# yjtang249/MIPSFusion

Measured on AMD Instinct MI355X. Metric: rays*samples/s per GPU, full optimisation iteration (fwd + bwd + pose+map Adam), 4096 rays x 64 samples, 640x480 RGB-D, higher is better.
Workload: dtype f32; decoder products as 3 x bf16 pieces of each fp32 operand, 6 bf16 MFMAs per product, fp32 accumulate; 1 GPU; BASELINE config 2: FastCaMo-synth apartment_2, 1 active submap per GPU, 4096 rays x 64 samples, hash grid 2^19 x 16 x 2, 620x460 synthetic RGB-D; rays=4096, samples_per_ray=64, hash_size=19, parallelism=single gpu

## Files before the change

include/mipsf.h:

```cpp
#ifndef MIPSF_H
#define MIPSF_H

#include <stdint.h>

#ifdef __cplusplus
extern "C" {
#endif

#define MIPSF_MAX_LEVELS 32
#define MIPSF_ABI_VERSION 2

const char* mipsf_last_error(void);
int mipsf_abi_version(void);
int mipsf_device_cu_count(void);

typedef struct mipsf_grid_meta {
    uint32_t n_levels;
    uint32_t n_features;
    uint32_t log2_hashmap_size;
    uint32_t base_resolution;
    float per_level_scale;
    float log2_per_level_scale;
    uint32_t n_params;
    uint32_t offsets[MIPSF_MAX_LEVELS + 1];
// ... 115 lines not shown
    uint32_t struct_size;
    uint32_t M;
    const float* packed16;
    const float* x;
    const float* out;
    const float* dout;
    const float* saved;
    float* dfeat;
    float* dx;
    float* dact;
    uint32_t* tile_live;
    int feat_layout;
    int flags;
    uint32_t packed16_floats;
    const uint32_t* live_list;
} mipsf_decoder_chain16_args;
int mipsf_decoder_bwd_chain16(const mipsf_decoder_chain16_args* args_host, void* stream);
#define MIPSF_WGRAD_LEAN_DACT 1u
#define MIPSF_WGRAD_DETERMINISTIC 2u
#define MIPSF_TILE_ORDER_MAX_M (1u << 27)
typedef struct mipsf_decoder_wgrad16_args {
    uint32_t struct_size;
    uint32_t M;
    const float* packed16;
    const float* feat;
    const float* x;
    const float* saved;
    const float* dact;
    const uint32_t* tile_live;
    const mipsf_decoder_grads* grads;
// ... 156 lines not shown
```

mipsfusion_amd/_lib.py:

```python
from __future__ import annotations

import ctypes as C
import os
from typing import Optional

import torch

_HERE = os.path.dirname(os.path.abspath(__file__))
LIB_PATH = os.environ.get("MIPSF_LIB") or os.path.join(_HERE, "libmipsf_hip.so")
MAX_LEVELS = 32
FEAT_AOS, FEAT_LEVEL_MAJOR = 0, 1
PREC = {"f32": 0, "f16x3": 1, "f16": 2, "bf16x3": 3, "bf16x6": 4}


class GridMeta(C.Structure):
    _fields_ = [("n_levels", C.c_uint32), ("n_features", C.c_uint32), ("log2_hashmap_size", C.c_uint32),
                ("base_resolution", C.c_uint32), ("per_level_scale", C.c_float),
                ("log2_per_level_scale", C.c_float), ("n_params", C.c_uint32),
                ("offsets", C.c_uint32 * (MAX_LEVELS + 1)), ("resolutions", C.c_uint32 * MAX_LEVELS),
                ("scales", C.c_float * MAX_LEVELS)]


class DecoderWeights(C.Structure):
    _fields_ = [(n, C.c_void_p) for n in ("w_pts0", "b_pts0", "w_pts2", "b_pts2", "w_rgb0", "b_rgb0",
# ... 21 lines not shown
        return a
    cls.new = staticmethod(new)
    return cls


_VP, _CU, _CI = C.c_void_p, C.c_uint32, C.c_int
HashgridBwdArgs = _args("HashgridBwdArgs", [("M", _CU), ("x", _VP), ("params", _VP), ("dout", _VP), ("dparams", _VP), ("dx", _VP),
                                            ("scratch", _VP), ("counters", _VP), ("meta", C.POINTER(GridMeta)),
                                            ("feat_layout", _CI), ("flags", _CU)])
DecoderFwd16Args = _args("DecoderFwd16Args", [("M", _CU), ("packed16", _VP), ("feat", _VP), ("x", _VP), ("out", _VP), ("saved", _VP),
                                              ("tile_live_clear", _VP), ("feat_layout", _CI), ("precision", _CI),
                                              ("sdf_only", _CI), ("lean_record", _CI), ("packed16_floats", _CU)])
DecoderChain16Args = _args("DecoderChain16Args", [("M", _CU), ("packed16", _VP), ("x", _VP), ("out", _VP), ("dout", _VP),
                                                  ("saved", _VP), ("dfeat", _VP), ("dx", _VP), ("dact", _VP), ("tile_live", _VP),
                                                  ("feat_layout", _CI), ("flags", _CI), ("packed16_floats", _CU),
                                                  ("live_list", _VP)])
DecoderWgrad16Args = _args("DecoderWgrad16Args", [("M", _CU), ("packed16", _VP), ("feat", _VP), ("x", _VP), ("saved", _VP),
                                                  ("dact", _VP), ("tile_live", _VP), ("grads", C.POINTER(DecoderGrads)),
                                                  ("partial", _VP), ("feat_layout", _CI), ("arithmetic", _CI), ("flags", _CU),
                                                  ("packed16_floats", _CU), ("live_list", _VP)])
RenderFwdArgs = _args("RenderFwdArgs", [("N", _CU), ("S", _CU), ("raw", _VP), ("z_vals", _VP), ("target_rgb", _VP), ("target_d", _VP),
                                        ("counts", _VP), ("cfg", C.POINTER(RenderCfg)), ("rgb", _VP), ("depth", _VP),
                                        ("depth_var", _VP), ("disp", _VP), ("acc", _VP), ("weights", _VP), ("losses", _VP),
                                        ("partial", _VP), ("loss_weights", _VP), ("loss_total", _VP), ("ticket", _VP),
                                        ("sums", _VP), ("draw", _VP)])
RenderBwdArgs = _args("RenderBwdArgs", [("N", _CU), ("S", _CU), ("N_norm", _CU), ("raw", _VP), ("z_vals", _VP), ("target_rgb", _VP),
                                        ("target_d", _VP), ("counts", _VP), ("losses", _VP), ("cfg", C.POINTER(RenderCfg)),
                                        ("g_losses", _VP), ("g_total", _VP), ("loss_weights", _VP), ("g_rgb", _VP),
                                        ("g_depth", _VP), ("draw", _VP), ("flags", _CU)])
RENDER_BWD_KEEP_IF_UNIT = 1

# ... 535 lines not shown
```

mipsfusion_amd/csrc/common.h:

```cpp
#pragma once
#include <hip/hip_runtime.h>
#include <stdint.h>
#include <stdarg.h>
#include <stdio.h>

#include "../../include/mipsf.h"
#include "../../include/mipsf_compact.h"

#define MIPSF_WAVE 64

namespace mipsf {

void set_error(const char* fmt, ...);
int check_launch(const char* what);

constexpr int MAX_DEVICES = 64;
inline int device_slot() {
    int d = 0;
    if (hipGetDevice(&d) != hipSuccess || d < 0 || d >= MAX_DEVICES) return 0;
    return d;
}
int device_cus();

uint64_t hashgrid_bwd_scratch_floats(const mipsf_grid_meta* meta, uint32_t M, int need_dx);
// ... 56 lines not shown
    }
    n.norm_factor = c.norm_factor;
    return n;
}

#if defined(__HIP_DEVICE_COMPILE__) && !defined(MIPSF_KEEP_PACKED_FP32)
#define MIPSF_SINGLE_FP32 __attribute__((target("no-packed-fp32-ops")))
#else
#define MIPSF_SINGLE_FP32
#endif

__device__ __forceinline__ float normalise1(float p, double sub, double div, double nf) {
    return (float)((((double)p - sub) / div) / nf);
}

__device__ __forceinline__ float wave_sum(float v) {
#pragma unroll
    for (int o = 32; o > 0; o >>= 1) v += __shfl_xor(v, o, 64);
    return v;
}
__device__ __forceinline__ double wave_sum_d(double v) {
#pragma unroll
    for (int o = 32; o > 0; o >>= 1) v += __shfl_xor(v, o, 64);
    return v;
}

__device__ __forceinline__ float sigmoidf_(float x) { return 1.0f / (1.0f + expf(-x)); }

}
```

mipsfusion_amd/csrc/decoder16.hip:

```cpp
#include "decoder_dev.h"
#include "launch.h"
#include <stdlib.h>

namespace mipsf {
using namespace dl;

typedef _Float16 h8 __attribute__((ext_vector_type(8)));
typedef _Float16 h2 __attribute__((ext_vector_type(2)));
typedef __bf16 bf8 __attribute__((ext_vector_type(8)));
typedef __bf16 bf2 __attribute__((ext_vector_type(2)));

__device__ __forceinline__ f32x16 mfma16(h8 a, h8 b, f32x16 c) {
    return __builtin_amdgcn_mfma_f32_32x32x16_f16(a, b, c, 0, 0, 0);
}
template <int NP>
__device__ __forceinline__ f32x16 mfmaP(h8 a, h8 b, f32x16 c) {
    if constexpr (NP == 3)
        return __builtin_amdgcn_mfma_f32_32x32x16_bf16(__builtin_bit_cast(bf8, a), __builtin_bit_cast(bf8, b), c, 0, 0, 0);
    else
        return __builtin_amdgcn_mfma_f32_32x32x16_f16(a, b, c, 0, 0, 0);
}

template <bool SPLIT>
__device__ __forceinline__ void split8(const float (&v)[8], h8& hi, h8& lo) {
// ... 752 lines not shown
    const uint32_t lo = wbits[2 * w], hi = wbits[2 * w + 1];
    const uint64_t s = (uint64_t)blockIdx.x * LC_BLOCK + t;
    const bool live = ((lane < 32 ? lo >> lane : hi >> (lane - 32)) & 1u) != 0u && s < M;
    pos += lane < 32 ? (uint32_t)__popc(lo & ((1u << lane) - 1u)) : (uint32_t)__popc(lo) + (uint32_t)__popc(hi & ((1u << (lane - 32)) - 1u));
    if (live) ll[MIPSF_LIVE_HEADER + pos] = (uint32_t)s;
    if (blockIdx.x == gridDim.x - 1) {
        uint32_t total = 0;
        for (uint32_t v = 0; v < LC_BLOCK / MIPSF_WAVE; ++v) total += wsum[v];
        for (uint32_t v = 0; v < LC_BLOCK / 32; ++v) total += (uint32_t)__popc(wbits[v]);
        const uint32_t padded = (total + 31u) & ~31u;
        if (t < padded - total) ll[MIPSF_LIVE_HEADER + total + t] = MIPSF_LIVE_PAD;
        if (t == 0) ll[0] = total, ll[1] = padded / 32u;
    }
}

template <int LAYOUT, int NP, bool COMPACT = false, typename Img>
__device__ __forceinline__ void decoder16_bwd_tile(const Img bimg, const float* __restrict__ x,
                                                   const float* __restrict__ out, const float* __restrict__ dout,
                                                   const float* __restrict__ saved, float* __restrict__ dfeat,
                                                   float* __restrict__ dx, float* __restrict__ dact,
                                                   float* __restrict__ dsmall, uint32_t M, int64_t tile, int lane_in,
                                                   uint32_t* __restrict__ tile_live = nullptr, bool lean_dact = false,
                                                   const uint32_t* __restrict__ live_idx = nullptr) {
    static_assert(NP == 2 || NP == 3, "the chain runs on split operands");
    int lane = lane_in;
    asm volatile("" : "+v"(lane));
    const int j = lane & 31, h = lane >> 5;
    const uint32_t s_raw = COMPACT ? live_idx[tile * 32 + j] : (uint32_t)(tile * 32 + j);
    const bool live = s_raw < M;
    const uint32_t s = live ? s_raw : M - 1;
    const uint32_t lane16 = 16u * (uint32_t)lane;
    const srd_t da = make_srd(dact ? dact + (size_t)tile * ACT_TILE_FLOATS : nullptr, dact ? ACT_TILE_FLOATS * 4 : 0);
    const srd_t da_opt = make_srd(dact ? dact + (size_t)tile * ACT_TILE_FLOATS : nullptr, (dact && !lean_dact) ? ACT_TILE_FLOATS * 4 : 0);

#ifdef D16_TRACE
    unsigned long long tr_t[12];
    const unsigned long long tr_w0 = wall_clock64();
#endif
// ... 29 lines not shown
    }
    D16_MARK(1);
    {
        const float2* o = reinterpret_cast<const float2*>(out + (size_t)s * 10);
#pragma unroll
        for (int c = 0; c < 5; ++c) o2[c] = o[c];
    }
#ifndef D16_BWD_X_LATE
    const float x0 = x[3 * (size_t)s], x1 = x[3 * (size_t)s + 1], x2 = x[3 * (size_t)s + 2];
#endif
    const uint2* mk = reinterpret_cast<const uint2*>(saved + (((size_t)M + 127) / 128) * 4 * ACT_TILE_FLOATS) +
                      (COMPACT ? (size_t)(s >> 5) * (MASK_TILE_WORDS / 2) + ((s & 31u) + 32u * (uint32_t)h)
                               : (size_t)tile * (MASK_TILE_WORDS / 2) + lane);
    const uint2 mk1 = mk[0], mk3 = mk[64];
    const uint32_t m1[2] = {mk1.x, mk1.y}, m3[2] = {mk3.x, mk3.y};

    D16_MARK(2);
    float dlg[N_CLASS], drgb[3];
    {
        const float gv[10] = {g2[0].x, g2[0].y, g2[1].x, g2[1].y, g2[2].x, g2[2].y, g2[3].x, g2[3].y, g2[4].x, g2[4].y};
        const float ov[10] = {o2[0].x, o2[0].y, o2[1].x, o2[1].y, o2[2].x, o2[2].y, o2[3].x, o2[3].y, o2[4].x, o2[4].y};
        const float g_sdf = live ? gv[3] : 0.f, g_ent = live ? gv[4] : 0.f;
        float p[N_CLASS], dp[N_CLASS], dot = 0.f;
#pragma unroll
        for (int c = 0; c < N_CLASS; ++c) {
            p[c] = ov[5 + c];
            const float q = p[c] + 1e-5f;
            const float dent = -1.0f * (log2f(q) + p[c] / (q * 0.69314718055994530942f));
            dp[c] = (live ? gv[5 + c] : 0.f) + g_sdf * (0.5f * (float)c) + g_ent * dent;
            dot += p[c] * dp[c];
// ... 36 lines not shown
        buf_store16_nosoff<D16_BWD_STORE_AUX>((mat == 2 || (mat == 1 && q >= 8)) ? da_opt : da, lane16, (mat * 16 + q) * 1024,
                           make_float4(acc[rt][4 * g] * down, acc[rt][4 * g + 1] * down, acc[rt][4 * g + 2] * down,
                                       acc[rt][4 * g + 3] * down));
    };

    D16_MARK(3);
    f32x16 dG3[4];
    mfma16_layer<RT16_S2T, T16_S2T, NP, INIT_ZERO>(bimg.at(OFF16B_S2T, OFF16B_S2T), lane, h, dG3,
        [&](int, h8 (&b)[3]) { b[0] = lgp[0], b[1] = lgp[1], b[2] = lgp[2]; });
#pragma unroll
    for (int rt = 0; rt < 4; ++rt)
#pragma unroll
        for (int r = 0; r < 16; ++r) dG3[rt][r] = mask_apply(m3, rt, r, dG3[rt][r] * acc_unscale<NP>());

    D16_MARK(4);
    f32x16 dIn3[3];
    mfma16_layer<RT16_B3, T16_B3, NP, INIT_ZERO>(bimg.at(OFF16B_B3, OFF16B_B3), lane, h, dIn3,
        [&](int t, h8 (&b)[3]) {
            float v[8];
#pragma unroll
            for (int u = 0; u < 8; ++u) v[u] = dG3[t >> 1][8 * (t & 1) + u];
            cut8<NP>(v, b);
        },
        [&](int t) {
            store_piece(2, dG3, 2 * t);
            store_piece(2, dG3, 2 * t + 1);
        });
#pragma unroll
    for (int rt = 0; rt < 3; ++rt)
#pragma unroll
        for (int r = 0; r < 16; ++r) dIn3[rt][r] = dIn3[rt][r] * acc_unscale<NP>();
    if (live) {
#pragma unroll
        for (int r = 0; r < 16; r += 2) {
            const int row = rowmap(r, h);
            const float2 v = make_float2(dIn3[2][r] * down, dIn3[2][r + 1] * down);
            if (LAYOUT == MIPSF_FEAT_AOS)
                *reinterpret_cast<float2*>(dfeat + (size_t)s * N_GRID + row) = v;
            else
                *reinterpret_cast<float2*>(dfeat + ((size_t)(row >> 1) * M + s) * 2) = v;
        }
    }

    D16_MARK(5);
    f32x16 dH2[4];
    dH2[0] = dIn3[0], dH2[1] = dIn3[1];
    {
        f32x16 dRgb[2];
        mfma16_layer<RT16_RGBT, T16_RGBT, NP, INIT_ZERO>(bimg.at(OFF16B_RGBT, OFF16B_RGBT), lane, h, dRgb,
            [&](int, h8 (&b)[3]) { b[0] = rgp[0], b[1] = rgp[1], b[2] = rgp[2]; });
        dH2[2] = dRgb[0] * acc_unscale<NP>(), dH2[3] = dRgb[1] * acc_unscale<NP>();
    }

    D16_MARK(6);
    f32x16 dG1[4];
    mfma16_layer<RT16_B2, T16_B2, NP, INIT_ZERO>(bimg.at(OFF16B_B2, OFF16B_B2), lane, h, dG1,
// ... 1 lines not shown
            float v[8];
#pragma unroll
            for (int u = 0; u < 8; ++u) v[u] = dH2[t >> 1][8 * (t & 1) + u];
            cut8<NP>(v, b);
        },
        [&](int t) {
            store_piece(1, dH2, 2 * t);
            store_piece(1, dH2, 2 * t + 1);
        });
#pragma unroll
    for (int rt = 0; rt < 4; ++rt)
#pragma unroll
        for (int r = 0; r < 16; ++r) dG1[rt][r] = mask_apply(m1, rt, r, dG1[rt][r] * acc_unscale<NP>());

    D16_MARK(7);
    f32x16 dE[2];
    mfma16_layer<RT16_B1, T16_B1, NP, INIT_ZERO>(bimg.at(OFF16B_B1, OFF16B_B1), lane, h, dE,
        [&](int t, h8 (&b)[3]) {
            if (t == 8) {
                b[0] = rgp[0], b[1] = rgp[1], b[2] = rgp[2];
            } else {
                float v[8];
#pragma unroll
                for (int u = 0; u < 8; ++u) v[u] = dG1[(t >> 1) & 3][8 * (t & 1) + u];
                cut8<NP>(v, b);
            }
        },
        [&](int t) {
            if (t < 8) {
                store_piece(0, dG1, 2 * t);
// ... 11 lines not shown
    float g3[3] = {0.f, 0.f, 0.f};
#pragma unroll
    for (int d = 0; d < 3; ++d) {
        const float xd = d == 0 ? x0 : (d == 1 ? x1 : x2);
#pragma unroll
        for (int k = 0; k < 8; ++k) {
            const float arg = fmaf(ldexpf(xd, k), PI_F, h ? HALF_PI_F : 0.0f);
            g3[d] = g3[d] + de[d * 8 + k] * ((ldexpf(1.0f, k) * PI_F) * cos_reduced(arg));
        }
    }
    g3[0] += h == 0 ? de[24] : 0.0f;
    g3[1] += h == 1 ? de[24] : 0.0f;
    g3[2] += h == 0 ? de[25] : 0.0f;
#pragma unroll
    for (int d = 0; d < 3; ++d) g3[d] = g3[d] + __shfl_xor(g3[d], 32, 64);
    if (live && h == 0) {
        dx[3 * (size_t)s] = g3[0], dx[3 * (size_t)s + 1] = g3[1], dx[3 * (size_t)s + 2] = g3[2];
    }
#ifdef D16_TRACE
    D16_MARK(9);
    if (lane == 0) {
        const unsigned w = (blockIdx.x * (blockDim.x >> 6) + (threadIdx.x >> 6)) & 4095u;
        for (int k = 0; k < 9; ++k) d16_trace[w * 16 + k] += tr_t[k + 1] - tr_t[k];
        d16_trace[w * 16 + 12] += wall_clock64() - tr_w0;
        d16_trace[w * 16 + 15] += 1ull;
    }
#endif
}

template <int LAYOUT, int NP, bool COMPACT>
__global__ __launch_bounds__(DEC_BLOCK, 2) void decoder16_bwd_kernel(const float* __restrict__ packed16,
                                                                     const float* __restrict__ x,
                                                                     const float* __restrict__ out,
                                                                     const float* __restrict__ dout,
                                                                     const float* __restrict__ saved,
                                                                     float* __restrict__ dfeat, float* __restrict__ dx,
                                                                     float* __restrict__ dact, float* __restrict__ dsmall,
                                                                     uint32_t M, uint32_t* __restrict__ tile_live, uint32_t lean_dact,
                                                                     const uint32_t* __restrict__ live_list) {
    const int lane = threadIdx.x & 63;
    const int64_t tile = (int64_t)blockIdx.x * (DEC_BLOCK / 64) + __builtin_amdgcn_readfirstlane((int)(threadIdx.x >> 6));
    if (tile * 32 >= (int64_t)M) return;
    if (COMPACT && tile >= (int64_t)live_list[1]) return;
    const ImgBuf bimg{make_srd(reinterpret_cast<const _Float16*>(packed16 + TAIL16_FLOATS) + OFF16_BWD_HALVES,
                               IMG16B_HALVES * 4), 0u, (uint32_t)IMG16B_HALVES * 2u, ext16_srd<NP>(packed16), (uint32_t)EXT16_BWD * 2u};
    decoder16_bwd_tile<LAYOUT, NP, COMPACT>(bimg, x, out, dout, saved, dfeat, dx, dact, dsmall, M, tile, lane, tile_live, lean_dact != 0u,
                                            COMPACT ? live_list + MIPSF_LIVE_HEADER : nullptr);
}

constexpr int B16_LDS_BYTES = IMG16B_HALVES * 4;
static_assert(B16_LDS_BYTES <= 160 * 1024, "the backward image sets must fit the LDS of a CU");
template <int LAYOUT, int NP, bool COMPACT>
__global__ __launch_bounds__(F16_LDS_BLOCK, 1) void decoder16_bwd_lds_kernel(const float* __restrict__ packed16,
                                                                             const float* __restrict__ x,
                                                                             const float* __restrict__ out,
                                                                             const float* __restrict__ dout,
                                                                             const float* __restrict__ saved,
                                                                             float* __restrict__ dfeat,
                                                                             float* __restrict__ dx,
                                                                             float* __restrict__ dact,
                                                                             float* __restrict__ dsmall, uint32_t M,
                                                                             uint32_t n_tiles_all,
                                                                             uint32_t* __restrict__ tile_live, uint32_t lean_dact,
                                                                             const uint32_t* __restrict__ live_list) {
    const uint32_t n_tiles = COMPACT ? (uint32_t)__builtin_amdgcn_readfirstlane((int)live_list[1]) : n_tiles_all;
    const uint32_t* live_idx = COMPACT ? live_list + MIPSF_LIVE_HEADER : nullptr;
    extern __shared__ __attribute__((aligned(16))) float4 wbuf[];
    lds_preload<F16_LDS_BLOCK>(wbuf, reinterpret_cast<const _Float16*>(packed16 + TAIL16_FLOATS) + OFF16_BWD_HALVES, B16_LDS_BYTES / 16);
    __syncthreads();
    const int lane = threadIdx.x & 63;
    constexpr uint32_t WPB = F16_LDS_BLOCK / 64;
    const uint32_t w = (uint32_t)__builtin_amdgcn_readfirstlane((int)(threadIdx.x >> 6));
    if (tile_live != nullptr && gridDim.x >= 8u) {
        const uint32_t q = blockIdx.x & 7u;
        uint32_t* counter = tile_live + 64 * q;
        for (;;) {
            uint32_t i = 0;
            if (lane == 0) i = atomicAdd(counter, 1u);
            i = (uint32_t)__builtin_amdgcn_readfirstlane((int)i);
            const uint32_t tile = (((i >> 3) * 8u + q) << 3) + (i & 7u);
            if ((tile & ~7u) >= n_tiles) break;
            if (tile >= n_tiles) continue;
            uint32_t z = 0;
            asm volatile("" : "+v"(z));
            const h8* imgp = reinterpret_cast<const h8*>(wbuf + z);
            decoder16_bwd_tile<LAYOUT, NP, COMPACT>(ImgLds{imgp, imgp + IMG16B_HALVES / 8, ext16_srd<NP>(packed16), (uint32_t)EXT16_BWD * 2u},
                                       x, out, dout, saved, dfeat, dx, dact, dsmall,
                                       M, (int64_t)tile, lane, tile_live, lean_dact != 0u, live_idx);
        }
        return;
    }
    uint32_t k = 0;
    for (uint32_t first = blockIdx.x * WPB; first < n_tiles; first += gridDim.x * WPB, ++k) {
        const uint32_t tile = first + ((w + k) & (WPB - 1));
        if (tile >= n_tiles) continue;
        uint32_t z = 0;
        asm volatile("" : "+v"(z));
        const h8* imgp = reinterpret_cast<const h8*>(wbuf + z);
        decoder16_bwd_tile<LAYOUT, NP, COMPACT>(ImgLds{imgp, imgp + IMG16B_HALVES / 8, ext16_srd<NP>(packed16), (uint32_t)EXT16_BWD * 2u},
                                   x, out, dout, saved, dfeat, dx, dact, dsmall, M,
                                   (int64_t)tile, lane, tile_live, lean_dact != 0u, live_idx);
    }
}

template <int NP>
__global__ __launch_bounds__(256) void decoder_pack16_kernel(W w, float* __restrict__ packed16) {
    const int idx = blockIdx.x * blockDim.x + threadIdx.x;
    uint16_t* ext = reinterpret_cast<uint16_t*>(packed16 + PACKED16_FLOATS);
    auto piece = [&](float v, int pl) -> uint16_t {
        if (NP == 3) return bf16_bits(bf16_piece(v, pl));
        const _Float16 hi = (_Float16)v;
        return __builtin_bit_cast(uint16_t, pl == 0 ? hi : (_Float16)(v - (float)hi));
    };
    if (NP == 3) {
        static_assert(OFF_BIAS - OFF_TRGB <= HEAD16_HALVES / 2, "the fp32 head tables fit the head region of the tail");
        if (idx < OFF_BIAS - OFF_TRGB) packed16[idx] = packed_value(w, OFF_TRGB + idx);
// ... 118 lines not shown
            }
            return check_launch("decoder_fwd16");
        };
        constexpr int_tag<(NP.value < 2 ? 2 : NP.value)> NP_LEAN;
        if (sdf_only) return arm(int_tag<0>{}, yes, NP);
        if (saved != nullptr && lean_record == 2) return arm(int_tag<3>{}, no, NP_LEAN);
        if (saved != nullptr && lean_record) return arm(int_tag<2>{}, no, NP_LEAN);
        if (saved != nullptr) return arm(int_tag<1>{}, no, NP);
        return arm(int_tag<0>{}, no, NP);
    }); });
}


int mipsf_decoder_bwd_chain16(const mipsf_decoder_chain16_args* a, void* stream) {
    MIPSF_REQUIRE(a != nullptr, "null argument block");
    MIPSF_REQUIRE(a->struct_size == sizeof(mipsf_decoder_chain16_args), "mipsf_decoder_chain16_args: struct_size %u, this library expects %u",
                  a->struct_size, (unsigned)sizeof(mipsf_decoder_chain16_args));
    const float* packed16 = a->packed16; const int feat_layout = a->feat_layout; const float* x = a->x; const float* out = a->out;
    const float* dout = a->dout; const float* saved = a->saved; float* dfeat = a->dfeat; float* dx = a->dx; float* dact = a->dact;
    uint32_t* tile_live = a->tile_live; const int flags = a->flags; const uint32_t M = a->M;
    const uint32_t* live_list = a->live_list;
    {
        const int fam = (flags & MIPSF_CHAIN_BF16X6) ? MIPSF_PREC_BF16X6 : MIPSF_PREC_F16X3;
        MIPSF_REQUIRE(a->packed16_floats == 0u || a->packed16_floats == decoder_packed16_floats(fam),
                      "packed16 holds %u floats, this chain needs %u: packed for the other family?", a->packed16_floats,
                      (unsigned)decoder_packed16_floats(fam));
    }
    if (M == 0) return 0;
    MIPSF_REQUIRE((flags & ~(MIPSF_CHAIN_HEADER_CLEAR | MIPSF_CHAIN_LEAN_DACT | MIPSF_CHAIN_BF16X6)) == 0, "unknown flags 0x%x", flags);
    const bool bf = (flags & MIPSF_CHAIN_BF16X6) != 0;
    const int header_is_clear = flags & MIPSF_CHAIN_HEADER_CLEAR;
    const uint32_t lean_dact = (flags & MIPSF_CHAIN_LEAN_DACT) ? 1u : 0u;
// ... 1 lines not shown
    MIPSF_REQUIRE(feat_layout == MIPSF_FEAT_AOS || feat_layout == MIPSF_FEAT_LEVEL_MAJOR, "bad layout");
    MIPSF_REQUIRE(live_list == nullptr || tile_live != nullptr, "the chain over a live-sample list deals its tiles through tile_live's header");
    const uint64_t n_bt = ((uint64_t)M + 127) / 128;
    const uint32_t blocks = (uint32_t)((((uint64_t)M + 31) / 32 + 3) / 4);
    float* dsmall = dact ? dact + n_bt * 4 * ACT_TILE_FLOATS : nullptr;
    hipStream_t s = (hipStream_t)stream;
    const uint32_t n_tiles = (uint32_t)(((uint64_t)M + 31) / 32);
    const int cus = device_cus();
    if (cus <= 0) return 3;
    const bool persistent = n_tiles >= (uint32_t)cus * persist_min_tiles_per_cu() && !getenv("MIPSF_B16_NO_LDS");
    if (tile_live != nullptr && !header_is_clear && hipMemsetAsync(tile_live, 0, TL_HEADER * sizeof(uint32_t), s) != hipSuccess) {
        set_error("cannot clear the tile counters");
        return 4;
    }
    return with_layout(feat_layout, [&](auto LAY) { return with_bool(bf, [&](auto BF) { return with_bool(live_list != nullptr, [&](auto CMP) {
        constexpr int NP = BF.value ? 3 : 2;
        if (persistent) {
            constexpr auto kern = decoder16_bwd_lds_kernel<LAY.value, NP, CMP.value>;
            if (!grant_lds<kern>(B16_LDS_BYTES)) return lds_refused(B16_LDS_BYTES);
            hipLaunchKernelGGL(kern, dim3(cus), dim3(F16_LDS_BLOCK), B16_LDS_BYTES, s, packed16, x, out, dout, saved, dfeat, dx, dact,
                               dsmall, M, n_tiles, tile_live, lean_dact, live_list);
        } else {
            hipLaunchKernelGGL((decoder16_bwd_kernel<LAY.value, NP, CMP.value>), dim3(blocks), dim3(DEC_BLOCK), 0, s, packed16, x, out,
                               dout, saved, dfeat, dx, dact, dsmall, M, tile_live, lean_dact, live_list);
        }
        return check_launch("decoder_bwd_chain16");
    }); }); });
}

int mipsf_decoder_live_compact(const float* dout, uint32_t M, uint32_t* live_list, float* dfeat, float* dx, int feat_layout,
                               void* stream) {
    MIPSF_REQUIRE(live_list != nullptr, "null live_list");
    MIPSF_REQUIRE(feat_layout == MIPSF_FEAT_AOS || feat_layout == MIPSF_FEAT_LEVEL_MAJOR, "bad layout");
    hipStream_t s = (hipStream_t)stream;
    if (M == 0) {
        if (hipMemsetAsync(live_list, 0, 2 * sizeof(uint32_t), s) != hipSuccess) {
            set_error("cannot clear the header of the live-sample list");
            return 4;
        }
        return 0;
    }
    MIPSF_REQUIRE(dout && dfeat && dx, "null pointer");
// ... 22 lines not shown
```

mipsfusion_amd/csrc/hashgrid.hip:

```cpp
#include "common.h"
#include "launch.h"
#include "decoder_layout.h"

namespace mipsf {

constexpr uint32_t P1 = 2654435761u;
constexpr uint32_t P2 = 805459861u;
constexpr int HG_BLOCK = 256;

struct Cell {
    uint32_t c[3];
    float f[3];
};

__device__ __forceinline__ Cell locate(const float* __restrict__ x, uint32_t i, float scale) {
    Cell r;
#pragma unroll
    for (int d = 0; d < 3; ++d) {
        const float pos = fmaf(scale, x[3 * (size_t)i + d], 0.5f);
        const float fl = floorf(pos);
        r.c[d] = (uint32_t)(int)fl;
        r.f[d] = pos - fl;
    }
    return r;
// ... 76 lines not shown
#pragma unroll
    for (int sub = 0; sub < 4; ++sub) {
        const int d0 = d == 0 ? 1 : 0;
        const int d1 = d == 2 ? 1 : 2;
        const int b0 = sub & 1, b1 = (sub >> 1) & 1;
        float wgt = scale;
        wgt = wgt * (b0 ? cell.f[d0] : 1.0f - cell.f[d0]);
        wgt = wgt * (b1 ? cell.f[d1] : 1.0f - cell.f[d1]);
        const int left = (b0 << d0) | (b1 << d1);
        const int right = left | (1 << d);
        s0 = s0 + wgt * (v[right].x - v[left].x);
        s1 = s1 + wgt * (v[right].y - v[left].y);
    }
}

__device__ __forceinline__ bool ray_wants_dx(const uint32_t* __restrict__ ray_mask, uint32_t S, uint32_t i) {
    return ray_mask == nullptr || ray_mask[S == 64u ? i >> 6 : i / S] != 0u;
}

template <int LAYOUT, bool JAC>
__global__ __launch_bounds__(HG_BLOCK) void hashgrid_fwd_kernel(const float* __restrict__ x,
                                                                const float2* __restrict__ table,
                                                                float* __restrict__ out, float* __restrict__ jac,
                                                                uint32_t M, GridLevels g, uint32_t nchunk,
                                                                const uint32_t* __restrict__ ray_mask, uint32_t S) {
    uint32_t chunk;
    const int level = decode_level(g.n_levels, nchunk, chunk);
    if (level >= (int)g.n_levels) return;
    const uint32_t i = chunk * HG_BLOCK + threadIdx.x;
    if (i >= M) return;

    const uint32_t off = g.offsets[level];
    const uint32_t size = g.offsets[level + 1] - off;
// ... 1542 lines not shown
```

mipsfusion_amd/model/scene_rep.py:

```python
import copy

import numpy as np
import os
import torch
import torch.nn as nn

from .. import ops
from .._lib import FEAT_LEVEL_MAJOR
from .decoder import MLP_reg
from .encodings import get_encoder


class _PlaceFn(torch.autograd.Function):

    @staticmethod
    def forward(ctx, rays_o, rays_d, target_d, noise, tables, rc, N, S):
        rays_o, rays_d = ops._f32c(rays_o), ops._f32c(rays_d)
        z_vals, xn, counts = ops.sample_rays(rays_o, rays_d, target_d, noise, tables, rc, N, S)
        ctx.rc, ctx.N, ctx.S = rc, N, S
        ctx.save_for_backward(z_vals)
        ctx.mark_non_differentiable(z_vals, counts)
        ctx.set_materialize_grads(False)
        return z_vals, xn, counts

# ... 78 lines not shown
        if ctx.tile_live is not None:
            saved.mipsf_tile_live = ctx.tile_live
        det = ops.resolve_deterministic(ctx.owner.deterministic)
        direct = ctx.owner.accumulate_param_grads_in_place and all(
            p.is_leaf and not p._backward_hooks for p in (grid_params, *weights))
        grads = None
        if need_w:
            grads = []
            for w, need in zip(weights, ctx.needs_input_grad[4:]):
                if direct and need:
                    if w.grad is None:
                        w.grad = torch.zeros_like(w)
                    grads.append(w.grad)
                else:
                    grads.append(torch.zeros_like(w))
        dfeat, dx, _, tiles = ops.decoder_bwd(packed, feat, FEAT_LEVEL_MAJOR, xn, None, out, ops._f32c(dout), saved, grads,
                                              ctx.M, precision=ctx.prec, packed16=packed if ctx.prec != "f32" else None,
                                              wgrad_precision=("stream_" + ctx.prec) if ctx.lean else ctx.owner.wgrad_precision,
                                              recompute_h1=ctx.lean, return_tiles=True, deterministic=det)
        dparams = None
        fresh_grad = False
        if need_g:
            if direct:
                if grid_params.grad is None:
                    grid_params.grad = torch.zeros_like(grid_params)
                    fresh_grad = True
                dparams = grid_params.grad
            else:
                dparams = torch.zeros_like(grid_params)
        if need_g:
            ops.hashgrid_bwd(xn, grid_params.detach(), dfeat, dparams, ctx.meta, FEAT_LEVEL_MAJOR, None, routed=ctx.routed,
                             dparams_zero=(not direct) or fresh_grad or ctx.owner.grid_grad_is_zero_at_backward, deterministic=det)
            ctx.routed = None
        if need_x:
# ... 63 lines not shown
    def __init__(self, config, bound_box, coords_norm_factor):
        super().__init__()
        self.config = config
        self.bounding_box = bound_box
        self.coords_norm_factor = coords_norm_factor
        self._bound64 = torch.as_tensor(bound_box).detach().to("cpu", torch.float64).tolist()
        self._half64 = torch.as_tensor(coords_norm_factor).detach().to("cpu", torch.float64).reshape(-1).tolist()
        self.accumulate_param_grads_in_place = False
        self.grid_grad_is_zero_at_backward = False
        self.deterministic = None
        self.decoder_precision = "bf16x6"
        self.wgrad_precision = "auto"
        self.lean_record = True
        self.route_ahead = False
        self.mask_fixed_rays = os.environ.get("MIPSF_NO_DX_MASK", "0") != "1"
        self.ray_share_reduce = None
        self._frozen_pack = None
        self._tables = {}
        self._jitter_ring = {}
        self.get_resolution()
        self.get_encoding(config)
        self.get_decoder(config)
        self.save_initial_param()

    def get_resolution(self):
        dim_max = max(b[1] - b[0] for b in self._bound64)
        if self.config["grid"]["voxel_sdf"] > 10:
            self.resolution_sdf = self.config["grid"]["voxel_sdf"]
        else:
            self.resolution_sdf = int(dim_max / self.config["grid"]["voxel_sdf"])
# ... 47 lines not shown
    def __deepcopy__(self, memo):
        with torch.random.fork_rng(devices=[]):
            new = JointEncoding(self.config, self.bounding_box, self.coords_norm_factor)
        memo[id(self)] = new
        dev = self.embed_fn.params.device
        new.to(dev)
        new.load_state_dict(self.state_dict())
        new.initial_dict = copy.deepcopy(self.initial_dict)
        new.accumulate_param_grads_in_place = self.accumulate_param_grads_in_place
        new.grid_grad_is_zero_at_backward = self.grid_grad_is_zero_at_backward
        new.decoder_precision = self.decoder_precision
        new.wgrad_precision = self.wgrad_precision
        new.lean_record = self.lean_record
        new.route_ahead = self.route_ahead
        new.mask_fixed_rays = self.mask_fixed_rays
        new.deterministic = self.deterministic
        new._frozen_pack = None
        new.train(self.training)
        return new

    def query_sdf(self, query_points):
        needs_grad = torch.is_grad_enabled() and (query_points.requires_grad or
                                                  any(p.requires_grad for p in self.parameters()))
        if needs_grad:
            return self.query_color_sdf(query_points)[..., 3:4]
        flat = torch.reshape(query_points, [-1, query_points.shape[-1]]) / self.config["training"]["norm_factor"]
        if not flat.is_cuda:
            raise RuntimeError("JointEncoding runs on the GPU only (no CPU fallback)")
        xn = ops._f32c(flat)
        prec = self.decoder_precision
# ... 132 lines not shown
```

mipsfusion_amd/ops.py:

```python
from __future__ import annotations

import ctypes as C
import os
from typing import Optional

import torch

from . import _lib
from ._lib import FEAT_AOS, FEAT_LEVEL_MAJOR, check, dptr, lib, stream_ptr

DECODER_PARAM_ORDER = ("pts_linear.0.weight", "pts_linear.0.bias", "pts_linear.2.weight", "pts_linear.2.bias",
                       "rgb_linear.0.weight", "rgb_linear.0.bias", "sdf_linear.0.weight", "sdf_linear.0.bias",
                       "sdf_linear.2.weight", "sdf_linear.2.bias")
_DEC_FIELDS = ("w_pts0", "b_pts0", "w_pts2", "b_pts2", "w_rgb0", "b_rgb0", "w_sdf0", "b_sdf0", "w_sdf2", "b_sdf2")
_DEC_SHAPES = ((128, 51), (128,), (128, 128), (128,), (3, 115), (3,), (128, 96), (128,), (5, 128), (5,))


PROFILE = None


class _timed:
    def __init__(self, name, stream=None):
        self.name, self.stream = name, stream

# ... 42 lines not shown
                                               stream_ptr()), "hashgrid_fwd (with the Jacobian)")
        return out, jac
    with _timed("hashgrid_fwd"):
        check(lib().mipsf_hashgrid_fwd(dptr(x), dptr(params), dptr(out), None, M, C.byref(meta), layout, stream_ptr()),
              "hashgrid_fwd")
    return out


class LiveList:
    __slots__ = ("buf",)

    def __init__(self, buf):
        self.buf = buf


def hashgrid_dx_from_jac(jac, dout, dx, meta, layout=FEAT_AOS, tiles=None, ray_mask=None):
    M = dx.shape[0]
    if ray_mask is not None:
        if ray_mask.shape[0] == 0 or M % ray_mask.shape[0] != 0:
            raise RuntimeError(f"ray mask: {M} samples are not whole rays of {ray_mask.shape[0]} rays")
        lst = isinstance(tiles, LiveList)
        with _timed("hashgrid_dx"):
            check(lib().mipsf_hashgrid_dx_from_jac_masked(dptr(jac), dptr(dout), dptr(dx),
                                                          None if lst else dptr(tiles, torch.int32),
                                                          dptr(tiles.buf, torch.int32) if lst else None,
                                                          dptr(ray_mask, torch.int32), M // ray_mask.shape[0], M,
                                                          C.byref(meta), layout, stream_ptr()), "hashgrid_dx_from_jac_masked")
        return
    if isinstance(tiles, LiveList):
        with _timed("hashgrid_dx"):
            check(lib().mipsf_hashgrid_dx_from_jac_list(dptr(jac), dptr(dout), dptr(dx), dptr(tiles.buf, torch.int32), M,
# ... 254 lines not shown
            saved.mipsf_lean_record = True
        if masks_only:
            saved.mipsf_masks_only = True
        if tile_live is not None:
            saved.mipsf_tile_live = [tile_live, True]
        return out, saved
    pe_mode = 0 if embed_pos is None else 1
    with _timed("decoder_fwd"):
        check(lib().mipsf_decoder_fwd(dptr(packed), dptr(feat), layout, dptr(x), dptr(embed_pos), pe_mode, dptr(out),
                                      dptr(saved), M, stream_ptr()), "decoder_fwd")
    return out, saved


def decoder_bwd(packed, feat, layout, x, embed_pos, out, dout, saved, grads, M, precision: str = "f32", packed16=None,
                wgrad_precision: str = "auto", recompute_h1: bool = False, return_tiles: bool = False,
                deterministic: bool = False):
    if wgrad_precision == "auto":
        wgrad_precision = ("stream_" + precision) if (precision in SPLIT_PRECISIONS and embed_pos is None) else "f32"
    if getattr(saved, "mipsf_masks_only", False) and grads is not None:
        raise RuntimeError("this activation record holds the ReLU masks only (decoder_fwd(save='masks')): no weight gradients")
    if getattr(saved, "mipsf_lean_record", False) and grads is not None:
        if wgrad_precision not in ("stream_f16x3", "stream_bf16x6") or packed16 is None or wgrad_precision != "stream_" + precision:
            raise RuntimeError("this activation record was saved lean (no H1): the weight gradients need the streaming kernel "
                               "of the forward's arithmetic (wgrad_precision='stream_f16x3' / 'stream_bf16x6') with packed16 "
                               "(H1 is recomputed from x)")
        recompute_h1 = True
    dev = x.device
    dfeat = torch.empty_like(feat)
    dx = torch.empty((M, 3), dtype=torch.float32, device=dev)
    dpe = torch.empty((M, 48), dtype=torch.float32, device=dev) if embed_pos is not None else None
    dact = None if (grads is None and precision in SPLIT_PRECISIONS) else torch.empty(_lib.buffer_size(_lib.SIZE_DECODER_DACT, M), dtype=torch.float32, device=dev)
# ... 15 lines not shown
                tile_live, hdr_clear = pre[0], hdr_clear | 1
                pre[1] = False
            else:
                tile_live = torch.empty(_lib.buffer_size(_lib.SIZE_DECODER_TILE_WORDS, M), dtype=torch.int32, device=dev)
            _LAST_TILE_LIVE = (tile_live, M, False)
            exchange = wgrad_precision == "stream_" + precision and recompute_h1 and packed16 is not None
            if (COMPACT_LIVE and (grads is None or exchange)
                    and _lib.buffer_size(_lib.SIZE_DECODER_SAVED, M) * 4 < (1 << 32)):
                live_list = torch.empty(_lib.buffer_size(_lib.SIZE_DECODER_LIVE_LIST, M), dtype=torch.int32, device=dev)
                _LAST_TILE_LIVE = (live_list, M, True)
                with _timed("decoder_bwd_chain"):
                    check(lib().mipsf_decoder_live_compact(dptr(dout), M, dptr(live_list, torch.int32), dptr(dfeat), dptr(dx),
                                                           layout, stream_ptr()), "decoder_live_compact")
        a = _lib.DecoderChain16Args.new(live_list=dptr(live_list, torch.int32), M=M, packed16=dptr(packed16), x=dptr(x), out=dptr(out), dout=dptr(dout), saved=dptr(saved),
                                        dfeat=dptr(dfeat), dx=dptr(dx), dact=dptr(dact), tile_live=dptr(tile_live, torch.int32),
                                        feat_layout=layout, flags=hdr_clear | (2 if lean_dact else 0), packed16_floats=packed16.numel())
        with _timed("decoder_bwd_chain"):
            check(lib().mipsf_decoder_bwd_chain16(C.byref(a), stream_ptr()), "decoder_bwd_chain16")
    else:
        with _timed("decoder_bwd_chain"):
            check(lib().mipsf_decoder_bwd_chain(dptr(packed), layout, dptr(x), pe_mode, dptr(out), dptr(dout),
                                                dptr(saved), dptr(dfeat), dptr(dx), dptr(dpe), dptr(dact), M,
                                                stream_ptr()), "decoder_bwd_chain")
    tiles = LiveList(live_list) if live_list is not None else tile_live
    if grads is not None:
        partial = torch.empty(_lib.buffer_size(_lib.SIZE_DECODER_WGRAD_PARTIAL), dtype=torch.float32, device=dev)
        st = _decoder_struct(grads, _lib.DecoderGrads)
        if wgrad_precision.startswith("stream_"):
            if embed_pos is not None:
                raise RuntimeError("the streaming weight-gradient kernel computes the positional encoding in-kernel")
            arith = _lib.PREC[wgrad_precision[len("stream_"):]]
            if recompute_h1 and (wgrad_precision not in ("stream_f16x3", "stream_bf16x6") or packed16 is None):
                raise RuntimeError("recompute_h1 needs wgrad_precision 'stream_f16x3' / 'stream_bf16x6' and packed16")
            if recompute_h1:
                _check_family(packed16, wgrad_precision[len("stream_"):])
            a = _lib.DecoderWgrad16Args.new(live_list=dptr(live_list, torch.int32),
                                            M=M, packed16=dptr(packed16) if recompute_h1 else None, feat=dptr(feat), x=dptr(x),
                                            saved=dptr(saved), dact=dptr(dact), tile_live=dptr(tile_live, torch.int32),
                                            grads=C.pointer(st), partial=dptr(partial), feat_layout=layout, arithmetic=arith,
# ... 463 lines not shown
```

Measured before the change: 447.8 million rays*samples/s.

## Fuse Jacobian position-gradient contraction into the 16-bit decoder backward chain

```diff
diff --git a/include/mipsf.h b/include/mipsf.h
--- a/include/mipsf.h
+++ b/include/mipsf.h
@@ -153,6 +153,9 @@
     int flags;
     uint32_t packed16_floats;
     const uint32_t* live_list;
+    const float* jac;
+    const uint32_t* ray_mask;
+    uint32_t samples_per_ray;
 } mipsf_decoder_chain16_args;
 int mipsf_decoder_bwd_chain16(const mipsf_decoder_chain16_args* args_host, void* stream);
 #define MIPSF_WGRAD_LEAN_DACT 1u
diff --git a/mipsfusion_amd/_lib.py b/mipsfusion_amd/_lib.py
--- a/mipsfusion_amd/_lib.py
+++ b/mipsfusion_amd/_lib.py
@@ -59,7 +59,8 @@
 DecoderChain16Args = _args("DecoderChain16Args", [("M", _CU), ("packed16", _VP), ("x", _VP), ("out", _VP), ("dout", _VP),
                                                   ("saved", _VP), ("dfeat", _VP), ("dx", _VP), ("dact", _VP), ("tile_live", _VP),
                                                   ("feat_layout", _CI), ("flags", _CI), ("packed16_floats", _CU),
-                                                  ("live_list", _VP)])
+                                                  ("live_list", _VP), ("jac", _VP), ("ray_mask", _VP),
+                                                  ("samples_per_ray", _CU)])
 DecoderWgrad16Args = _args("DecoderWgrad16Args", [("M", _CU), ("packed16", _VP), ("feat", _VP), ("x", _VP), ("saved", _VP),
                                                   ("dact", _VP), ("tile_live", _VP), ("grads", C.POINTER(DecoderGrads)),
                                                   ("partial", _VP), ("feat_layout", _CI), ("arithmetic", _CI), ("flags", _CU),
diff --git a/mipsfusion_amd/csrc/common.h b/mipsfusion_amd/csrc/common.h
--- a/mipsfusion_amd/csrc/common.h
+++ b/mipsfusion_amd/csrc/common.h
@@ -94,6 +94,10 @@
     return (float)((((double)p - sub) / div) / nf);
 }
 
+__device__ __forceinline__ bool ray_wants_dx(const uint32_t* __restrict__ ray_mask, uint32_t S, uint32_t i) {
+    return ray_mask == nullptr || ray_mask[S == 64u ? i >> 6 : i / S] != 0u;
+}
+
 __device__ __forceinline__ float wave_sum(float v) {
 #pragma unroll
     for (int o = 32; o > 0; o >>= 1) v += __shfl_xor(v, o, 64);
diff --git a/mipsfusion_amd/csrc/decoder16.hip b/mipsfusion_amd/csrc/decoder16.hip
--- a/mipsfusion_amd/csrc/decoder16.hip
+++ b/mipsfusion_amd/csrc/decoder16.hip
@@ -790,14 +790,22 @@
     }
 }
 
-template <int LAYOUT, int NP, bool COMPACT = false, typename Img>
+__device__ __forceinline__ float half_to_both(float v, int half) {
+    const uint32_t u = __builtin_bit_cast(uint32_t, v);
+    const auto r = __builtin_amdgcn_permlane32_swap(u, u, false, false);
+    return __builtin_bit_cast(float, half ? r[1] : r[0]);
+}
+
+template <int LAYOUT, int NP, bool COMPACT = false, bool DXJ = false, typename Img>
 __device__ __forceinline__ void decoder16_bwd_tile(const Img bimg, const float* __restrict__ x,
                                                    const float* __restrict__ out, const float* __restrict__ dout,
                                                    const float* __restrict__ saved, float* __restrict__ dfeat,
                                                    float* __restrict__ dx, float* __restrict__ dact,
                                                    float* __restrict__ dsmall, uint32_t M, int64_t tile, int lane_in,
                                                    uint32_t* __restrict__ tile_live = nullptr, bool lean_dact = false,
-                                                   const uint32_t* __restrict__ live_idx = nullptr) {
+                                                   const uint32_t* __restrict__ live_idx = nullptr,
+                                                   const float* __restrict__ jac = nullptr,
+                                                   const uint32_t* __restrict__ ray_mask = nullptr, uint32_t S = 0) {
     static_assert(NP == 2 || NP == 3, "the chain runs on split operands");
     int lane = lane_in;
     asm volatile("" : "+v"(lane));
@@ -857,6 +865,7 @@
                                : (size_t)tile * (MASK_TILE_WORDS / 2) + lane);
     const uint2 mk1 = mk[0], mk3 = mk[64];
     const uint32_t m1[2] = {mk1.x, mk1.y}, m3[2] = {mk3.x, mk3.y};
+    const bool wants_dx = !DXJ || ray_wants_dx(ray_mask, S, s);
 
     D16_MARK(2);
     float dlg[N_CLASS], drgb[3];
@@ -923,6 +932,21 @@
         for (int r = 0; r < 16; ++r) dG3[rt][r] = mask_apply(m3, rt, r, dG3[rt][r] * acc_unscale<NP>());
 
     D16_MARK(4);
+    float2 jl[DXJ ? 8 : 1][3];
+    if (DXJ) {
+#pragma unroll
+        for (int i = 0; i < 8; ++i)
+#pragma unroll
+            for (int d = 0; d < 3; ++d) jl[i][d] = make_float2(0.f, 0.f);
+        if (live && wants_dx) {
+#pragma unroll
+            for (int i = 0; i < 8; ++i) {
+                const float2* j2 = reinterpret_cast<const float2*>(jac) + (size_t)(rowmap(2 * i, h) >> 1) * 3 * M + s;
+#pragma unroll
+                for (int d = 0; d < 3; ++d) jl[i][d] = j2[(size_t)d * M];
+            }
+        }
+    }
     f32x16 dIn3[3];
     mfma16_layer<RT16_B3, T16_B3, NP, INIT_ZERO>(bimg.at(OFF16B_B3, OFF16B_B3), lane, h, dIn3,
         [&](int t, h8 (&b)[3]) {
@@ -939,16 +963,37 @@
     for (int rt = 0; rt < 3; ++rt)
 #pragma unroll
         for (int r = 0; r < 16; ++r) dIn3[rt][r] = dIn3[rt][r] * acc_unscale<NP>();
+    float2 gl[DXJ ? 8 : 1];
     if (live) {
 #pragma unroll
         for (int r = 0; r < 16; r += 2) {
             const int row = rowmap(r, h);
             const float2 v = make_float2(dIn3[2][r] * down, dIn3[2][r + 1] * down);
+            if (DXJ) gl[r >> 1] = v;
             if (LAYOUT == MIPSF_FEAT_AOS)
                 *reinterpret_cast<float2*>(dfeat + (size_t)s * N_GRID + row) = v;
             else
                 *reinterpret_cast<float2*>(dfeat + ((size_t)(row >> 1) * M + s) * 2) = v;
         }
+    } else if (DXJ) {
+#pragma unroll
+        for (int i = 0; i < 8; ++i) gl[i] = make_float2(0.f, 0.f);
+    }
+    if (DXJ) {
+        float ja[3] = {0.f, 0.f, 0.f};
+#pragma unroll
+        for (int i = 0; i < 8; i += 2) {
+#pragma unroll
+            for (int half = 0; half < 2; ++half) {
+#pragma unroll
+                for (int d = 0; d < 3; ++d) {
+                    ja[d] = ja[d] + (jl[i][d].x * gl[i].x + jl[i][d].y * gl[i].y);
+                    ja[d] = ja[d] + (jl[i + 1][d].x * gl[i + 1].x + jl[i + 1][d].y * gl[i + 1].y);
+                    ja[d] = half_to_both(ja[d], half);
+                }
+            }
+        }
+        if (live && wants_dx && h == 0) dx[3 * (size_t)s] = ja[0], dx[3 * (size_t)s + 1] = ja[1], dx[3 * (size_t)s + 2] = ja[2];
     }
 
     D16_MARK(5);
@@ -980,6 +1025,8 @@
         for (int r = 0; r < 16; ++r) dG1[rt][r] = mask_apply(m1, rt, r, dG1[rt][r] * acc_unscale<NP>());
 
     D16_MARK(7);
+    float ja[3] = {0.f, 0.f, 0.f};
+    if (DXJ && live && wants_dx && h == 0) ja[0] = dx[3 * (size_t)s], ja[1] = dx[3 * (size_t)s + 1], ja[2] = dx[3 * (size_t)s + 2];
     f32x16 dE[2];
     mfma16_layer<RT16_B1, T16_B1, NP, INIT_ZERO>(bimg.at(OFF16B_B1, OFF16B_B1), lane, h, dE,
         [&](int t, h8 (&b)[3]) {
@@ -1021,6 +1068,10 @@
     g3[2] += h == 0 ? de[25] : 0.0f;
 #pragma unroll
     for (int d = 0; d < 3; ++d) g3[d] = g3[d] + __shfl_xor(g3[d], 32, 64);
+    if (DXJ) {
+#pragma unroll
+        for (int d = 0; d < 3; ++d) g3[d] = wants_dx ? g3[d] + ja[d] : 0.0f;
+    }
     if (live && h == 0) {
         dx[3 * (size_t)s] = g3[0], dx[3 * (size_t)s + 1] = g3[1], dx[3 * (size_t)s + 2] = g3[2];
     }
@@ -1035,7 +1086,7 @@
 #endif
 }
 
-template <int LAYOUT, int NP, bool COMPACT>
+template <int LAYOUT, int NP, bool COMPACT, bool DXJ>
 __global__ __launch_bounds__(DEC_BLOCK, 2) void decoder16_bwd_kernel(const float* __restrict__ packed16,
                                                                      const float* __restrict__ x,
                                                                      const float* __restrict__ out,
@@ -1044,20 +1095,22 @@
                                                                      float* __restrict__ dfeat, float* __restrict__ dx,
                                                                      float* __restrict__ dact, float* __restrict__ dsmall,
                                                                      uint32_t M, uint32_t* __restrict__ tile_live, uint32_t lean_dact,
-                                                                     const uint32_t* __restrict__ live_list) {
+                                                                     const uint32_t* __restrict__ live_list,
+                                                                     const float* __restrict__ jac,
+                                                                     const uint32_t* __restrict__ ray_mask, uint32_t S) {
     const int lane = threadIdx.x & 63;
     const int64_t tile = (int64_t)blockIdx.x * (DEC_BLOCK / 64) + __builtin_amdgcn_readfirstlane((int)(threadIdx.x >> 6));
     if (tile * 32 >= (int64_t)M) return;
     if (COMPACT && tile >= (int64_t)live_list[1]) return;
     const ImgBuf bimg{make_srd(reinterpret_cast<const _Float16*>(packed16 + TAIL16_FLOATS) + OFF16_BWD_HALVES,
                                IMG16B_HALVES * 4), 0u, (uint32_t)IMG16B_HALVES * 2u, ext16_srd<NP>(packed16), (uint32_t)EXT16_BWD * 2u};
-    decoder16_bwd_tile<LAYOUT, NP, COMPACT>(bimg, x, out, dout, saved, dfeat, dx, dact, dsmall, M, tile, lane, tile_live, lean_dact != 0u,
-                                            COMPACT ? live_list + MIPSF_LIVE_HEADER : nullptr);
+    decoder16_bwd_tile<LAYOUT, NP, COMPACT, DXJ>(bimg, x, out, dout, saved, dfeat, dx, dact, dsmall, M, tile, lane, tile_live,
+                                                 lean_dact != 0u, COMPACT ? live_list + MIPSF_LIVE_HEADER : nullptr, jac, ray_mask, S);
 }
 
 constexpr int B16_LDS_BYTES = IMG16B_HALVES * 4;
 static_assert(B16_LDS_BYTES <= 160 * 1024, "the backward image sets must fit the LDS of a CU");
-template <int LAYOUT, int NP, bool COMPACT>
+template <int LAYOUT, int NP, bool COMPACT, bool DXJ>
 __global__ __launch_bounds__(F16_LDS_BLOCK, 1) void decoder16_bwd_lds_kernel(const float* __restrict__ packed16,
                                                                              const float* __restrict__ x,
                                                                              const float* __restrict__ out,
@@ -1069,7 +1122,9 @@
                                                                              float* __restrict__ dsmall, uint32_t M,
                                                                              uint32_t n_tiles_all,
                                                                              uint32_t* __restrict__ tile_live, uint32_t lean_dact,
-                                                                             const uint32_t* __restrict__ live_list) {
+                                                                             const uint32_t* __restrict__ live_list,
+                                                                             const float* __restrict__ jac,
+                                                                             const uint32_t* __restrict__ ray_mask, uint32_t S) {
     const uint32_t n_tiles = COMPACT ? (uint32_t)__builtin_amdgcn_readfirstlane((int)live_list[1]) : n_tiles_all;
     const uint32_t* live_idx = COMPACT ? live_list + MIPSF_LIVE_HEADER : nullptr;
     extern __shared__ __attribute__((aligned(16))) float4 wbuf[];
@@ -1091,9 +1146,9 @@
             uint32_t z = 0;
             asm volatile("" : "+v"(z));
             const h8* imgp = reinterpret_cast<const h8*>(wbuf + z);
-            decoder16_bwd_tile<LAYOUT, NP, COMPACT>(ImgLds{imgp, imgp + IMG16B_HALVES / 8, ext16_srd<NP>(packed16), (uint32_t)EXT16_BWD * 2u},
+            decoder16_bwd_tile<LAYOUT, NP, COMPACT, DXJ>(ImgLds{imgp, imgp + IMG16B_HALVES / 8, ext16_srd<NP>(packed16), (uint32_t)EXT16_BWD * 2u},
                                        x, out, dout, saved, dfeat, dx, dact, dsmall,
-                                       M, (int64_t)tile, lane, tile_live, lean_dact != 0u, live_idx);
+                                       M, (int64_t)tile, lane, tile_live, lean_dact != 0u, live_idx, jac, ray_mask, S);
         }
         return;
     }
@@ -1104,9 +1159,9 @@
         uint32_t z = 0;
         asm volatile("" : "+v"(z));
         const h8* imgp = reinterpret_cast<const h8*>(wbuf + z);
-        decoder16_bwd_tile<LAYOUT, NP, COMPACT>(ImgLds{imgp, imgp + IMG16B_HALVES / 8, ext16_srd<NP>(packed16), (uint32_t)EXT16_BWD * 2u},
+        decoder16_bwd_tile<LAYOUT, NP, COMPACT, DXJ>(ImgLds{imgp, imgp + IMG16B_HALVES / 8, ext16_srd<NP>(packed16), (uint32_t)EXT16_BWD * 2u},
                                    x, out, dout, saved, dfeat, dx, dact, dsmall, M,
-                                   (int64_t)tile, lane, tile_live, lean_dact != 0u, live_idx);
+                                   (int64_t)tile, lane, tile_live, lean_dact != 0u, live_idx, jac, ray_mask, S);
     }
 }
 
@@ -1255,8 +1310,16 @@
 
 int mipsf_decoder_bwd_chain16(const mipsf_decoder_chain16_args* a, void* stream) {
     MIPSF_REQUIRE(a != nullptr, "null argument block");
-    MIPSF_REQUIRE(a->struct_size == sizeof(mipsf_decoder_chain16_args), "mipsf_decoder_chain16_args: struct_size %u, this library expects %u",
-                  a->struct_size, (unsigned)sizeof(mipsf_decoder_chain16_args));
+    const bool has_dx_fields = a->struct_size == sizeof(mipsf_decoder_chain16_args);
+    MIPSF_REQUIRE(has_dx_fields || a->struct_size == offsetof(mipsf_decoder_chain16_args, jac),
+                  "mipsf_decoder_chain16_args: struct_size %u, this library expects %u (or %u: the block without jac)", a->struct_size,
+                  (unsigned)sizeof(mipsf_decoder_chain16_args), (unsigned)offsetof(mipsf_decoder_chain16_args, jac));
+    const float* jac = has_dx_fields ? a->jac : nullptr;
+    const uint32_t* ray_mask = has_dx_fields ? a->ray_mask : nullptr;
+    const uint32_t S = has_dx_fields ? a->samples_per_ray : 0u;
+    MIPSF_REQUIRE(ray_mask == nullptr || jac != nullptr, "ray_mask without jac: the mask belongs to the Jacobian's part of d x");
+    MIPSF_REQUIRE(ray_mask == nullptr || S != 0u, "ray_mask with samples_per_ray == 0");
+    MIPSF_REQUIRE(ray_mask == nullptr || a->M % S == 0u, "ray_mask: %u samples are not whole rays of %u", a->M, S);
     const float* packed16 = a->packed16; const int feat_layout = a->feat_layout; const float* x = a->x; const float* out = a->out;
     const float* dout = a->dout; const float* saved = a->saved; float* dfeat = a->dfeat; float* dx = a->dx; float* dact = a->dact;
     uint32_t* tile_live = a->tile_live; const int flags = a->flags; const uint32_t M = a->M;
@@ -1288,18 +1351,19 @@
         return 4;
     }
     return with_layout(feat_layout, [&](auto LAY) { return with_bool(bf, [&](auto BF) { return with_bool(live_list != nullptr, [&](auto CMP) {
+    return with_bool(jac != nullptr, [&](auto DXJ) {
         constexpr int NP = BF.value ? 3 : 2;
         if (persistent) {
-            constexpr auto kern = decoder16_bwd_lds_kernel<LAY.value, NP, CMP.value>;
+            constexpr auto kern = decoder16_bwd_lds_kernel<LAY.value, NP, CMP.value, DXJ.value>;
             if (!grant_lds<kern>(B16_LDS_BYTES)) return lds_refused(B16_LDS_BYTES);
             hipLaunchKernelGGL(kern, dim3(cus), dim3(F16_LDS_BLOCK), B16_LDS_BYTES, s, packed16, x, out, dout, saved, dfeat, dx, dact,
-                               dsmall, M, n_tiles, tile_live, lean_dact, live_list);
+                               dsmall, M, n_tiles, tile_live, lean_dact, live_list, jac, ray_mask, S);
         } else {
-            hipLaunchKernelGGL((decoder16_bwd_kernel<LAY.value, NP, CMP.value>), dim3(blocks), dim3(DEC_BLOCK), 0, s, packed16, x, out,
-                               dout, saved, dfeat, dx, dact, dsmall, M, tile_live, lean_dact, live_list);
+            hipLaunchKernelGGL((decoder16_bwd_kernel<LAY.value, NP, CMP.value, DXJ.value>), dim3(blocks), dim3(DEC_BLOCK), 0, s, packed16,
+                               x, out, dout, saved, dfeat, dx, dact, dsmall, M, tile_live, lean_dact, live_list, jac, ray_mask, S);
         }
         return check_launch("decoder_bwd_chain16");
-    }); }); });
+    }); }); }); });
 }
 
 int mipsf_decoder_live_compact(const float* dout, uint32_t M, uint32_t* live_list, float* dfeat, float* dx, int feat_layout,
diff --git a/mipsfusion_amd/csrc/hashgrid.hip b/mipsfusion_amd/csrc/hashgrid.hip
--- a/mipsfusion_amd/csrc/hashgrid.hip
+++ b/mipsfusion_amd/csrc/hashgrid.hip
@@ -114,9 +114,6 @@
     }
 }
 
-__device__ __forceinline__ bool ray_wants_dx(const uint32_t* __restrict__ ray_mask, uint32_t S, uint32_t i) {
-    return ray_mask == nullptr || ray_mask[S == 64u ? i >> 6 : i / S] != 0u;
-}
 
 template <int LAYOUT, bool JAC>
 __global__ __launch_bounds__(HG_BLOCK) void hashgrid_fwd_kernel(const float* __restrict__ x,
diff --git a/mipsfusion_amd/model/scene_rep.py b/mipsfusion_amd/model/scene_rep.py
--- a/mipsfusion_amd/model/scene_rep.py
+++ b/mipsfusion_amd/model/scene_rep.py
@@ -116,10 +116,12 @@
                     grads.append(w.grad)
                 else:
                     grads.append(torch.zeros_like(w))
+        chain_dx = need_x and ctx.prec in ops.SPLIT_PRECISIONS and not ctx.owner.dx_launch
         dfeat, dx, _, tiles = ops.decoder_bwd(packed, feat, FEAT_LEVEL_MAJOR, xn, None, out, ops._f32c(dout), saved, grads,
                                               ctx.M, precision=ctx.prec, packed16=packed if ctx.prec != "f32" else None,
                                               wgrad_precision=("stream_" + ctx.prec) if ctx.lean else ctx.owner.wgrad_precision,
-                                              recompute_h1=ctx.lean, return_tiles=True, deterministic=det)
+                                              recompute_h1=ctx.lean, return_tiles=True, deterministic=det,
+                                              jac=jac if chain_dx else None, ray_mask=ctx.ray_mask if chain_dx else None)
         dparams = None
         fresh_grad = False
         if need_g:
@@ -213,6 +215,7 @@
         self.lean_record = True
         self.route_ahead = False
         self.mask_fixed_rays = os.environ.get("MIPSF_NO_DX_MASK", "0") != "1"
+        self.dx_launch = os.environ.get("MIPSF_DX_LAUNCH", "0") == "1"
         self.ray_share_reduce = None
         self._frozen_pack = None
         self._tables = {}
@@ -290,6 +293,7 @@
         new.lean_record = self.lean_record
         new.route_ahead = self.route_ahead
         new.mask_fixed_rays = self.mask_fixed_rays
+        new.dx_launch = self.dx_launch
         new.deterministic = self.deterministic
         new._frozen_pack = None
         new.train(self.training)
diff --git a/mipsfusion_amd/ops.py b/mipsfusion_amd/ops.py
--- a/mipsfusion_amd/ops.py
+++ b/mipsfusion_amd/ops.py
@@ -80,7 +80,16 @@
         self.buf = buf
 
 
+class DxFormed:
+    __slots__ = ("tiles",)
+
+    def __init__(self, tiles):
+        self.tiles = tiles
+
+
 def hashgrid_dx_from_jac(jac, dout, dx, meta, layout=FEAT_AOS, tiles=None, ray_mask=None):
+    if isinstance(tiles, DxFormed):
+        return
     M = dx.shape[0]
     if ray_mask is not None:
         if ray_mask.shape[0] == 0 or M % ray_mask.shape[0] != 0:
@@ -365,7 +374,18 @@
 
 def decoder_bwd(packed, feat, layout, x, embed_pos, out, dout, saved, grads, M, precision: str = "f32", packed16=None,
                 wgrad_precision: str = "auto", recompute_h1: bool = False, return_tiles: bool = False,
-                deterministic: bool = False):
+                deterministic: bool = False, jac=None, ray_mask=None, samples_per_ray=None):
+    if jac is not None and precision not in SPLIT_PRECISIONS:
+        raise RuntimeError("decoder_bwd(jac=) belongs to the 16-bit chain: behind the fp32 decoder call hashgrid_dx_from_jac")
+    if ray_mask is not None:
+        if jac is None:
+            raise RuntimeError("decoder_bwd: ray_mask without jac")
+        if samples_per_ray is None:
+            if ray_mask.shape[0] == 0 or M % ray_mask.shape[0] != 0:
+                raise RuntimeError(f"ray mask: {M} samples are not whole rays of {ray_mask.shape[0]} rays")
+            samples_per_ray = M // ray_mask.shape[0]
+    if jac is not None and (jac.dim() != 4 or tuple(jac.shape) != (16, 3, M, 2)):
+        raise RuntimeError(f"decoder_bwd: jac has shape {tuple(jac.shape)}, the chain reads [16, 3, {M}, 2]")
     if wgrad_precision == "auto":
         wgrad_precision = ("stream_" + precision) if (precision in SPLIT_PRECISIONS and embed_pos is None) else "f32"
     if getattr(saved, "mipsf_masks_only", False) and grads is not None:
@@ -411,7 +431,9 @@
                                                            layout, stream_ptr()), "decoder_live_compact")
         a = _lib.DecoderChain16Args.new(live_list=dptr(live_list, torch.int32), M=M, packed16=dptr(packed16), x=dptr(x), out=dptr(out), dout=dptr(dout), saved=dptr(saved),
                                         dfeat=dptr(dfeat), dx=dptr(dx), dact=dptr(dact), tile_live=dptr(tile_live, torch.int32),
-                                        feat_layout=layout, flags=hdr_clear | (2 if lean_dact else 0), packed16_floats=packed16.numel())
+                                        feat_layout=layout, flags=hdr_clear | (2 if lean_dact else 0), packed16_floats=packed16.numel(),
+                                        jac=dptr(jac), ray_mask=dptr(ray_mask, torch.int32),
+                                        samples_per_ray=samples_per_ray or 0)
         with _timed("decoder_bwd_chain"):
             check(lib().mipsf_decoder_bwd_chain16(C.byref(a), stream_ptr()), "decoder_bwd_chain16")
     else:
@@ -420,6 +442,8 @@
                                                 dptr(saved), dptr(dfeat), dptr(dx), dptr(dpe), dptr(dact), M,
                                                 stream_ptr()), "decoder_bwd_chain")
     tiles = LiveList(live_list) if live_list is not None else tile_live
+    if jac is not None:
+        tiles = DxFormed(tiles)
     if grads is not None:
         partial = torch.empty(_lib.buffer_size(_lib.SIZE_DECODER_WGRAD_PARTIAL), dtype=torch.float32, device=dev)
         st = _decoder_struct(grads, _lib.DecoderGrads)
```

New measurement: 455.2 million rays*samples/s, median of 6. Within noise of the previous version (+1.7%).
